# jgillick/genesis-forge

Hardware: AMD Instinct MI355X
Metric: env-steps/sec (higher is better)
Workload: dtype f32; 1 GPU; go2_12dof_full_manager_stack; num_envs_per_gpu=65536, global_num_envs=65536, dofs=12, reward_terms=6, termination_terms=2, command_managers=1, obs_width=48, scene=synthetic (gf_synth_scene_step), parallelism=env-shard x1, hsa_enable_ipc_mode_legacy=0, setup_steps_before_warmup=8, fused_post_physics=True, observation_output=fresh

## Files before the change

### genesis-forge_amd/csrc/gf_post.hip

```cpp
#include <dlfcn.h>

#include <atomic>
#include <cstdio>
#include <cstdlib>
#include <cstring>
#include <mutex>

#include "gf_post_args.h"
#include "gf_post_ws.h"
#include "gf_post_programs.h"

namespace gf {

static int cmd_slot_of_reward_op(int op) {
    switch (op) {
        case GF_R_CMD_TRACK_LIN_VEL:
        case GF_R_CMD_TRACK_ANG_VEL:
        case GF_R_STAND_STILL: return 0;
        case GF_R_FEET_AIR_TIME: return 1;
        default: return -1;
    }
}
static bool reward_op_has_contact(int op) { return op == GF_R_HAS_CONTACT || op == GF_R_CONTACT_FORCE || op == GF_R_FEET_AIR_TIME || op == GF_R_FEET_SLIDE; }
static bool term_op_has_contact(int op) { return op == GF_T_HAS_CONTACT || op == GF_T_CONTACT_FORCE || op == GF_T_CONTACT_FORCE_GRACE; }
// ... 506 lines not shown
    if (num_mgr > 0) {
        UNSUP(!post_program_folds(pk.a));
        rc = fold_contacts(pk, mgrs, num_mgr);
        if (rc) return rc;
    }
    return post_launch(pk.a, s);
}

}

extern "C" __attribute__((visibility("default"))) int gf_post_physics_check(const GfPostRefs* r) {
    gf::Packer pk;
    return gf::pack(r, pk);
}

using gf::lds_ws_floats;

namespace {
constexpr int kDynBase = 100, kDynMax = 256;
struct DynProgram {
    void* dl;
    char name[64];
    int (*matches)(const gf::GfPostArgs*);
    const void* kernel;
    size_t (*lds_bytes)(int, int);
    bool folds;
};
DynProgram g_dyn[kDynMax];
std::atomic<int> g_dyn_count{0};
std::mutex g_dyn_mutex;
// ... 93 lines not shown
#else
    const gf::GfPostArgs& a = packed;
#endif
    int omax = 0;
    for (int m = 0; m < a.n_obs; ++m) omax = a.obs[m].width > omax ? a.obs[m].width : omax;
    const size_t fold_lds = a.cfold.num_mgr > 0 ? gf::fold_lds_bytes(a.cfold.num_contacts) : 0;
    auto with_fold = [&](size_t bytes, bool interp) {
        const size_t need = fold_lds ? fold_lds + (interp ? sizeof(gf::GfPostArgs) : 0) : 0;
        return (bytes > need ? bytes : need) + (size_t)gf::kWsTilesLdsFloats * sizeof(float);
    };
    const unsigned grid = gf::env_grid(a.num_envs);
    if (prog < 0) prog = select_program(a);
    if (tick) {
        const dim3 tg(grid + (unsigned)tick->upkeep), tb(gf::kWsBlock);
#define GF_RUN_TICK(P, interp) \
        gf::klaunch(gf::post_ws_kernel_tick<P>, tg, tb, with_fold((interp ? sizeof(gf::GfPostArgs) : 0) + lds_ws_floats<P>(omax, a.n_gait) * sizeof(float), interp), s, a, *tick->act, *tick->scene, tick->upkeep)
        if (prog == 1) GF_RUN_TICK(gf::ProgGo2CommandDirection, false);
        else if (prog == 2) GF_RUN_TICK(gf::ProgGo2Simple, false);
        else if (a.num_dofs == 12) GF_RUN_TICK(GF_TICK_INTERP(3), true);
        else GF_RUN_TICK(GF_TICK_INTERP(7), true);
#undef GF_RUN_TICK
        return gf::launch_status();
    }
    gf::PhaseScope scope(GF_PHASE_POST, s);
    if (prog >= kDynBase) {
        const DynProgram& d = g_dyn[prog - kDynBase];
        const size_t lds_dyn = with_fold(d.lds_bytes(omax, a.n_gait), false);
        void* kargs[1] = {const_cast<gf::GfPostArgs*>(&a)};
        if (scope.active()) {
            scope.use_dispatch_events();
            (void)hipExtLaunchKernel(d.kernel, dim3(grid), dim3(gf::kWsBlock), kargs, lds_dyn, s, scope.start(), scope.stop(), 0);
// ... 80 lines not shown
```

### genesis-forge_amd/csrc/gf_post_programs.h

```cpp
#pragma once

#include "gf_post_ws.h"

namespace gf {

struct ProgGo2CommandDirection {
    static constexpr bool kStatic = true;
    static constexpr const char* name = "go2_command_direction";
    static constexpr int DV = 3;
    static constexpr int n_term = 2;
    static constexpr TermSig term[n_term] = {{GF_T_TIMEOUT, GF_TERM_FLAG_TIME_OUT}, {GF_T_BAD_ORIENTATION, 0}};
    static constexpr int n_rew = 6;
    static constexpr RewSig rew[n_rew] = {{GF_R_BASE_HEIGHT, 0, 0, 0},       {GF_R_CMD_TRACK_LIN_VEL, 0, 0, 0}, {GF_R_CMD_TRACK_ANG_VEL, 0, 0, 2},
                                          {GF_R_LIN_VEL_Z_L2, 0, 0, 0},      {GF_R_ACTION_RATE_L2, 0, 0, 0},    {GF_R_DOF_SIMILAR_TO_DEFAULT, 0, 0, 0}};
    static constexpr int n_cmd = 1;
    static constexpr int cmd_width[GF_POST_MAX_CMD] = {3, 0};
    static constexpr int n_obs = 1;
    static constexpr int obs_width[GF_POST_MAX_OBS] = {48, 0};
    static constexpr int obs_history[GF_POST_MAX_OBS] = {1, 0};
    static constexpr int obs_items[GF_POST_MAX_OBS] = {7, 0};
    static constexpr ItemSig item[GF_POST_MAX_OBS][kPostMaxItems] = {{{GF_O_COMMAND, 3, 0, false, false},
                                                                      {GF_O_ANG_VEL_BODY, 3, 0, false, false},
                                                                      {GF_O_LIN_VEL_BODY, 3, 0, false, false},
                                                                      {GF_O_PROJ_GRAVITY, 3, 0, false, false},
// ... 197 lines not shown
    static constexpr int n_cmd = 2;
    static constexpr int cmd_width[GF_POST_MAX_CMD] = {3, 1};
    static constexpr int n_obs = 2;
    static constexpr int obs_width[GF_POST_MAX_OBS] = {94, 61};
    static constexpr int obs_history[GF_POST_MAX_OBS] = {3, 1};
    static constexpr int obs_items[GF_POST_MAX_OBS] = {7, 4};
    static constexpr ItemSig item[GF_POST_MAX_OBS][kPostMaxItems] = {
        {{1, 1, 1, false, true}, {1, 3, 0, false, true}, {2, 3, 0, true, true}, {4, 3, 0, false, true}, {5, 28, 0, false, true}, {6, 28, 0, true, true}, {8, 28, 0, false, true}},
        {{10, 2, 1, true, false}, {3, 3, 0, false, false}, {7, 28, 0, false, false}, {9, 28, 0, false, false}}};
    static constexpr int n_air = 2;
    static constexpr int n_gait = 0;
};

template <class P>
inline size_t lds_ws_floats(int omax, int n_gait) {
    return (size_t)(x_fields(n_gait) + ws_sum_rows<P>() + ws_aux_rows<P>() + ws_pre_rows<P>() + ws_obs_norm_rows<P>()) * kEnvBlock + (size_t)(omax + 1) * kEnvBlock;
}

template <class P>
bool program_matches(const GfPostArgs& a) {
    if ((a.term_done != 0) != prog_term_done<P>::value || a.num_dofs != 4 * P::DV || a.num_term != P::n_term || (a.num_rew < 0 ? 0 : a.num_rew) != P::n_rew || a.n_cmd != P::n_cmd || a.n_obs != P::n_obs || a.n_air != P::n_air ||
        a.n_gait != P::n_gait)
        return false;
    for (int k = 0; k < P::n_term; ++k)
        if (a.tterms[k].op != P::term[k].op || a.tterms[k].flags != P::term[k].flags) return false;
    for (int k = 0; k < P::n_rew; ++k) {
        const GfTerm& t = a.rterms[k];
        if (t.op != P::rew[k].op || t.flags != P::rew[k].flags || t.i[0] != P::rew[k].i0 || t.i[1] != P::rew[k].i1) return false;
    }
    for (int c = 0; c < P::n_cmd; ++c)
        if (a.cmds[c].width != P::cmd_width[c]) return false;
// ... 42 lines not shown
```

### genesis-forge_amd/csrc/gf_post_ws.h

```cpp
#pragma once

#include <utility>

#include "gf_obs_hist.h"
#include "gf_post_args.h"
#include "gf_scene_tile.h"

namespace gf {

static_assert(kObsBlock == 4 * kEnvBlock, "the history helpers assume the 4-wave workgroup");
constexpr int kWsBlock = 4 * kEnvBlock;
enum : int { X_TERM = 0, X_TRUNC = 1, X_DONE = 2, X_BLIN = 3, X_BANG = 6, X_GRAV = 9, X_CMD = 12, X_DIRTY = 20, X_FIELDS = 21,
             X_GAIT = X_FIELDS  };
__host__ __device__ constexpr int x_fields(int n_gait) { return X_FIELDS + (n_gait > 0 ? GF_GAIT_ROW : 0); }

struct TermSig { int op, flags; };
struct RewSig { int op, flags, i0, i1; };
struct ItemSig { int op, width, i0; bool scaled, noisy; };

template <class P, class = void>
struct prog_term_done : std::false_type {};
template <class P>
struct prog_term_done<P, std::void_t<decltype(P::term_done)>> : std::bool_constant<P::term_done> {};

template <int DV_, bool TAIL_ = false>
struct Interp {
    static constexpr bool kStatic = false;
    static constexpr int DV = DV_;
    static constexpr bool kTail = TAIL_;
};

template <class P>
struct WithTick : P {
    static constexpr bool kTick = true;
};
template <class P, class = void>
struct prog_tick : std::false_type {};
template <class P>
struct prog_tick<P, std::void_t<decltype(P::kTick)>> : std::bool_constant<P::kTick> {};

template <class F, int... I>
__device__ __forceinline__ void static_for_impl(F&& f, std::integer_sequence<int, I...>) {
    (f(std::integral_constant<int, I>{}), ...);
}
template <int N, class F>
__device__ __forceinline__ void static_for(F&& f) {
    static_for_impl(f, std::make_integer_sequence<int, N>{});
}

template <class P>
__device__ __forceinline__ const GfPostArgs& pick_args(const GfPostArgs& k, const float* l) {
    if constexpr (P::kStatic) return k;
    else return *reinterpret_cast<const GfPostArgs*>(l);
}
// ... 73 lines not shown
}
template <class P>
__host__ __device__ constexpr bool ws_prog_folds() {
    if constexpr (P::kStatic) {
        if (P::n_term == 0 && P::n_rew == 0 && P::n_cmd == 0 && P::n_gait == 0) return false;
        if (P::n_air > 0) return true;
        for (int k = 0; k < P::n_term; ++k)
            if (term_op_counts_contacts(P::term[k].op)) return true;
        for (int k = 0; k < P::n_rew; ++k)
            if (reward_op_reads_contacts(P::rew[k].op)) return true;
        return ws_obs_has<P>(GF_O_CONTACT_FORCE_NORM);
    } else {
        return true;
    }
}

#ifndef GF_WS_AHEAD
#define GF_WS_AHEAD 0
#endif
constexpr int kWsTilesLdsFloats = GF_WS_AHEAD > 0 ? 4 * kEnvBlock : 0;

template <class P>
__device__ __forceinline__ void post_ws_body(const GfPostArgs& karg, const GfActionArgs* const tick_act, const GfSynthSceneArgs* const tick_scene,
                                             const int tick_upkeep) {
    constexpr int DV = P::DV;
    constexpr bool kTick = prog_tick<P>::value;
    unsigned ws_block = blockIdx.x;
    if constexpr (kTick) {
        if ((int)blockIdx.x < tick_upkeep) {
            action_upkeep(*tick_act, tick_upkeep, kWsBlock);
// ... 43 lines not shown
        n_term = P::n_term; n_rew = P::n_rew; n_cmd = P::n_cmd; n_obs = P::n_obs;
    } else {
        n_term = UNI(a.num_term); n_rew = UNI(a.num_rew); n_cmd = UNI(a.n_cmd); n_obs = UNI(a.n_obs);
    }
    const uint64_t seed = UNI(a.seed);
    const bool obs_only = UNI(a.obs_only) != 0;
    constexpr int R = DV;
    const uint32_t ro = e * (uint32_t)D;
    GfStepStats* const k_stats = UNI(a.stats);
    GfStepStats* shard = k_stats ? stats_shard(k_stats) : nullptr;
    const bool logging = UNI(a.logging) != 0;
    float* const k_sums = UNI(a.episode_sums);
    float* const k_reward = UNI(a.reward);
    const bool has_reward = n_rew >= 0 && k_reward != nullptr;
    const float4 z4 = make_float4(0.f, 0.f, 0.f, 0.f);
    if constexpr (kTick) {
        static_assert(GF_WS_AHEAD == 0, "the look-ahead experiment would pull rows of a tile whose tick has not run into this CU's L1");
        static_assert(kSynthTileBlock == kWsBlock && 3 * 3 * kEnvBlock <= X_FIELDS * kEnvBlock, "the tick's workgroup and LDS fit the kernel's");
        const GfSynthSceneArgs& sc = *tick_scene;
        const int rows = (int)((int64_t)sc.num_envs - n0 < kEnvBlock ? (int64_t)sc.num_envs - n0 : kEnvBlock);
        float (&s3)[3][kEnvBlock * 3] = *reinterpret_cast<float (*)[3][kEnvBlock * 3]>(xch);
        SynthBase ticked;
        synth_tick_tile<DV, kEnvBlock, true>(sc, *tick_act, n0, rows, s3, ticked);
        GF_WSTAMP(12);
        __syncthreads();
        GF_WSTAMP(13);
    }
#if GF_WS_AHEAD > 0
    {
        const int64_t next_id = tile_id + GF_WS_AHEAD;
        if (next_id < (N + kEnvBlock - 1) / kEnvBlock) {
            const int64_t n2 = next_id * kEnvBlock + lane;
            const uint32_t e2 = (uint32_t)(n2 < N ? n2 : N - 1), ro2 = e2 * (uint32_t)D;
            float* const pf = lds + kArgVec * 4 + wave * kEnvBlock;
            auto warm = [&](const bool on, const float* base, const uint32_t off) GF_INLINE_LAMBDA {
                __builtin_amdgcn_global_load_lds(gsel(on, base, off), pf, 4, 0, 0);
            };
            if (wave == 0) {
// ... 145 lines not shown
    int& gait_sel = ctl.gait_sel; int& gait_resampled = ctl.gait_resampled;
    if (wave == 0) {
        q = make_float4(1.f, 0.f, 0.f, 0.f);
        ep_len = 0; term = 0; trunc = 0;
#pragma unroll
        for (int j = 0; j < GF_GAIT_ROW; ++j) grow[j] = 0.f;
        gait_sel = 0; gait_resampled = 0;
        ctl.log_bits = 0u; ctl.gait_logged = 0;
    } else {
#pragma unroll
        for (int c = 0; c < DV; ++c) { r_a[c] = z4; r_b[c] = z4; r_c[c] = z4; }
    }

    float fold_w[kSumRows > 0 ? kSumRows : 1];
    int32_t fold_row[kSumRows > 0 ? kSumRows : 1];
    if (wave == 0) {
        q = ldg4(gsel((needs & PN_QUAT) != 0, UNI(a.quat), 4u * e));
        const GF_GLOBAL float* pp = gsel((needs & PN_POS) != 0, UNI(a.pos), 3u * e);
        const GF_GLOBAL float* lp = gsel((needs & PN_LIN) != 0, UNI(a.lin_vel), 3u * e);
        const GF_GLOBAL float* ap = gsel((needs & PN_ANG) != 0, UNI(a.ang_vel), 3u * e);
        const V3 pos{pp[0], pp[1], pp[2]};
        const V3 lin{lp[0], lp[1], lp[2]}, ang{ap[0], ap[1], ap[2]};
        ep_len = *gsel((needs & PN_EPLEN) != 0, UNI(a.episode_length), e);
        const int max_len = *gsel((needs & PN_MAXLEN) != 0, UNI(a.max_episode_length), e);
#pragma unroll
        for (int c = 0; c < GF_POST_MAX_CMD; ++c) {
            const bool on = c < n_cmd;
            const uint32_t w = on ? (uint32_t)UNI(cmd_row(c).width) : 0u;
            const GF_GLOBAL float* cp = gsel(on, on ? UNI(a.cmds[c].command) : nullptr, e * w);
#pragma unroll
            for (int j = 0; j < kPostMaxRanges; ++j) cmd[c][j] = cp[(uint32_t)j < w ? j : 0];
        }
        if (has_gait) {
            const GF_GLOBAL float* gp = G(UNI(a.gait.state)) + (int64_t)e * GF_GAIT_ROW;
            const float4 g0 = ldg4(gp), g1 = ldg4(gp + 4), g2 = ldg4(gp + 8), g3 = ldg4(gp + 12);
            grow[0] = g0.x; grow[1] = g0.y; grow[2] = g0.z; grow[3] = g0.w; grow[4] = g1.x; grow[5] = g1.y; grow[6] = g1.z; grow[7] = g1.w;
            grow[8] = g2.x; grow[9] = g2.y; grow[10] = g2.z; grow[11] = g2.w; grow[12] = g3.x; grow[13] = g3.y; grow[14] = g3.z; grow[15] = g3.w;
            gait_sel = (int)G(UNI(a.gait.selected))[e];
// ... 133 lines not shown
#pragma unroll
            for (int j = 0; j < kPostMaxRanges; ++j) xch[(X_CMD + c * kPostMaxRanges + j) * kEnvBlock + lane] = cmd[c][j];
        xch[X_DIRTY * kEnvBlock + lane] = (float)((cmd_dirty[0] ? 1 : 0) | (cmd_dirty[1] ? 2 : 0));
    } else if (wave == 1) {
        if (logging) {
            if constexpr (P::kStatic) {
                static_for<P::n_rew>([&](auto K) GF_INLINE_LAMBDA {
                    constexpr int k_ = decltype(K)::value;
                    __builtin_amdgcn_global_load_lds(k_sums + (int64_t)karg.rterms[k_].row * N + n, lds_sums + k_ * kEnvBlock, 4, 0, 0);
                });
            } else {
                for (int k = 0; k < n_rew; ++k)
                    __builtin_amdgcn_global_load_lds(k_sums + (int64_t)uni(a.rterms[k].row) * N + n, lds_sums + k * kEnvBlock, 4, 0, 0);
            }
        }
        const GF_GLOBAL float* p0 = gsel((needs & PN_DOFDEV) != 0, UNI(a.dof_pos), ro);
        const GF_GLOBAL float* p1 = gsel((needs & PN_ACTRATE) != 0, UNI(a.env_actions), ro);
        const GF_GLOBAL float* p2 = gsel((needs & PN_ACTRATE) != 0, UNI(a.env_last_actions), ro);
        const GF_GLOBAL float* p3 = gsel((needs & PN_DOFDEV) != 0, UNI(a.default_dof_pos), 0u);
        float4 r_def[R];
        row_load<DV>(r_a, p0, D); row_load<DV>(r_b, p1, D); row_load<DV>(r_c, p2, D); row_load<DV>(r_def, p3, D);
        const GF_GLOBAL float* pp = gsel((needs & PN_POS) != 0, UNI(a.pos), 3u * e);
        const V3 pos{pp[0], pp[1], pp[2]};
        float4 qb = make_float4(1.f, 0.f, 0.f, 0.f);
        V3 wlin{0.f, 0.f, 0.f}, wang{0.f, 0.f, 0.f};
        if constexpr (ws_rew_body_frame<P>()) {
            qb = ldg4(gsel((needs & PN_QUAT) != 0, UNI(a.quat), 4u * e));
            const GF_GLOBAL float* lp = gsel((needs & PN_LIN) != 0, UNI(a.lin_vel), 3u * e);
            const GF_GLOBAL float* ap = gsel((needs & PN_ANG) != 0, UNI(a.ang_vel), 3u * e);
            wlin = V3{lp[0], lp[1], lp[2]};
            wang = V3{ap[0], ap[1], ap[2]};
        }
        const float* k_secs = UNI(a.episode_seconds);
        const float secs_in = *gsel(has_reward && k_secs != nullptr, k_secs, e);
        float dof_dev = 0.f, act_rate = 0.f, cmd0[3];
        {
            const float* v0 = UNI(a.command[0].command);
            const bool nv = v0 != nullptr;
            const uint32_t w = nv ? (uint32_t)UNI(a.command[0].width) : 0u;
            const uint32_t st = nv ? (uint32_t)(UNI(a.command[0].stride) ? UNI(a.command[0].stride) : UNI(a.command[0].width)) : 0u;
            const GF_GLOBAL float* cp = gsel(nv, v0, e * st);
// ... 46 lines not shown
                });
            }
        }
        rew.pos = pos;
        rew.dof_dev = dof_dev; rew.act_rate = act_rate; rew.secs_in = secs_in;
        rew.cmd0[0] = cmd0[0]; rew.cmd0[1] = cmd0[1]; rew.cmd0[2] = cmd0[2];
        if constexpr (P::kStatic) {
            static_for<P::n_rew>([&](auto K) GF_INLINE_LAMBDA {
                constexpr int k_ = decltype(K)::value;
                rew.vals[k_] = vals[k_];
                fold_w[k_] = karg.rterms[k_].w; fold_row[k_] = karg.rterms[k_].row;
                asm volatile("" : "+s"(fold_w[k_]), "+s"(fold_row[k_]));
            });
        }
    } else if (wave == 2) {
        const GF_GLOBAL float* p0 = gsel((needs & PN_DOFPOS) != 0, UNI(a.dof_pos), ro);
        const GF_GLOBAL float* p1 = gsel((needs & PN_DOFVEL) != 0, UNI(a.dof_vel), ro);
        const float* k_def = UNI(a.default_dof_pos);
        const GF_GLOBAL float* p2 = gsel(k_def != nullptr, k_def, 0u);
        row_load<DV>(r_a, p0, D); row_load<DV>(r_b, p1, D); row_load<DV>(r_c, p2, D);
        GF_WSTAMP(9);
        if constexpr (kPreRows > 0) {
            RewardRegs rp;
            rp.pos = V3{0.f, 0.f, 0.f}; rp.blin = rp.pos; rp.bang = rp.pos; rp.grav = rp.pos;
            rp.dof_dev = 0.f; rp.act_rate = 0.f; rp.terminated = 0;
            rp.cmd0[0] = 0.f; rp.cmd0[1] = 0.f; rp.cmd0[2] = 0.f;
            rp.n = n; rp.live = live;
            static_for<P::n_rew>([&](auto K) GF_INLINE_LAMBDA {
                constexpr int k_ = decltype(K)::value;
                if constexpr (reward_op_memory_only(P::rew[k_].op)) {
                    GfTerm t = karg.rterms[k_];
                    t.op = P::rew[k_].op; t.flags = P::rew[k_].flags; t.i[0] = P::rew[k_].i0; t.i[1] = P::rew[k_].i1;
                    lds_pre[ws_pre_slot<P>(k_) * kEnvBlock + lane] = eval_reward_term(t, a, rp);
                }
            });
        }
    } else {
        const GF_GLOBAL float* p0 = gsel((needs & PN_TARGETS) != 0, UNI(a.targets), ro);
        const GF_GLOBAL float* p1 = gsel((needs & PN_ACTIONS) != 0, UNI(a.env_actions), ro);
        row_load<DV>(r_a, p0, D); row_load<DV>(r_b, p1, D);
        if constexpr (P::kStatic && ws_obs_has<P>(GF_O_DOF_FORCE)) {
            row_load<DV>(r_c, gsel(UNI(a.dof_force) != nullptr, UNI(a.dof_force), ro), D);
        }
        if constexpr (kNormRows > 0) {
            static_for<P::n_obs>([&](auto M) GF_INLINE_LAMBDA {
                constexpr int m_ = decltype(M)::value;
                static_for<P::obs_items[m_]>([&](auto I) GF_INLINE_LAMBDA {
                    constexpr int i_ = decltype(I)::value;
                    if constexpr (P::item[m_][i_].op == GF_O_CONTACT_FORCE_NORM) {
                        const GfContactView cv = a.contact[P::item[m_][i_].i0];
                        const GF_GLOBAL float* r = G(cv.contacts) + n * cv.num_links * 3;
#pragma unroll
                        for (int l = 0; l < P::item[m_][i_].width; ++l)
                            lds_norm[(ws_obs_norm_slot<P>(m_, i_) + l) * kEnvBlock + lane] = norm3(r[3 * l], r[3 * l + 1], r[3 * l + 2]);
                    }
// ... 473 lines not shown
```

### genesis-forge_amd/csrc/gf_scene_tile.h

```cpp
#pragma once

#include "gf_action_row.h"

namespace gf {

struct SynthBase {
    float p[3], q[4], v[3], w[3];
};

struct SynthDraws {
    U4 b0, b1;
};
__device__ __forceinline__ SynthDraws synth_draws(const GfSynthSceneArgs& a, const uint32_t genv) {
    return SynthDraws{philox4x32_10(genv, 0u, (uint32_t)a.tick, (uint32_t)(a.tick >> 32), (uint32_t)a.seed, (uint32_t)(a.seed >> 32)),
                      philox4x32_10(genv, 1u, (uint32_t)a.tick, (uint32_t)(a.tick >> 32), (uint32_t)a.seed, (uint32_t)(a.seed >> 32))};
}

__device__ __forceinline__ void synth_base_math(const GfSynthSceneArgs& a, const float4 q4, const V3 w0, const V3 v0, const V3 p0,
                                                const SynthDraws& r, SynthBase& out) {
    const float dt = a.dt;
    const U4 b0 = r.b0, b1 = r.b1;
    const float s[6] = {u24_to_unit(b0.x) * 2.0f - 1.0f, u24_to_unit(b0.y) * 2.0f - 1.0f, u24_to_unit(b0.z) * 2.0f - 1.0f,
                        u24_to_unit(b0.w) * 2.0f - 1.0f, u24_to_unit(b1.x) * 2.0f - 1.0f, u24_to_unit(b1.y) * 2.0f - 1.0f};
    float w[3] = {w0.x, w0.y, w0.z}, v[3] = {v0.x, v0.y, v0.z}, p[3] = {p0.x, p0.y, p0.z};
// ... 18 lines not shown
    for (int j = 0; j < 3; ++j) { out.w[j] = w[j]; out.v[j] = v[j]; out.p[j] = p[j]; }
#pragma unroll
    for (int j = 0; j < 4; ++j) out.q[j] = nq[j];
}

__device__ __forceinline__ void synth_joint(float t, float& p, float& v, float rate, float dt) {
    v = (t - p) * rate;
    p = p + v * dt;
}

constexpr int kSynthTileBlock = 256;
constexpr int kSynthDofLanes = kSynthTileBlock - GF_WAVE;

__device__ __forceinline__ void wave_lds_sync() { __builtin_amdgcn_wave_barrier(); }

template <int DV, int TE, bool FOLD = false>
__device__ __forceinline__ void synth_dof_tile(const GfSynthSceneArgs& a, const GfActionArgs& act, const int64_t n0, const int rows, const int t) {
    const float dt = a.dt, rate = a.joint_rate;
    if constexpr (FOLD) {
        static_assert(DV > 0, "the fold moves float4s");
        constexpr int kIt = (TE * (DV > 0 ? DV : 1) + kSynthDofLanes - 1) / kSynthDofLanes;
        const int cnt = rows * DV;
        const int64_t f0 = n0 * DV;
        const float4* x4 = reinterpret_cast<const float4*>(act.actions_in) + f0;
        const bool keep = act.env_actions != nullptr;
        float4* e4 = reinterpret_cast<float4*>(keep ? act.env_actions : act.targets) + f0;
        float4* l4 = reinterpret_cast<float4*>(keep ? act.env_last_actions : act.targets) + f0;
        float4* t4 = reinterpret_cast<float4*>(act.targets) + f0;
        float4* p4 = reinterpret_cast<float4*>(a.dof_pos) + f0;
        float4* v4 = reinterpret_cast<float4*>(a.dof_vel) + f0;
        const int mode = act.mode;
        int flags = 0;
// ... 15 lines not shown
            if constexpr (!kConstsFirst) c0 = action_consts4(act, 4 * ((i < cnt ? i : cnt - 1) % DV), mode);
            float4 last, actions, tg;
            int fl = 0;
            action_row4(act, c0, mode, x[k], pv[k], last, actions, tg, fl);
            float4 v, p = dp[k];
            synth_joint(tg.x, p.x, v.x, rate, dt);
            synth_joint(tg.y, p.y, v.y, rate, dt);
            synth_joint(tg.z, p.z, v.z, rate, dt);
            synth_joint(tg.w, p.w, v.w, rate, dt);
            if (i < cnt) {
                flags |= fl;
                if (keep) { l4[i] = last; e4[i] = actions; }
                t4[i] = tg;
                v4[i] = v;
                p4[i] = p;
            }
        }
        action_flags_commit(act, flags);
    } else if (DV > 0) {
        constexpr int kIt = DV > 0 ? (TE * DV + kSynthDofLanes - 1) / kSynthDofLanes : 1;
        const int cnt = rows * DV;
        const float4* t4 = reinterpret_cast<const float4*>(a.targets) + n0 * DV;
        float4* p4 = reinterpret_cast<float4*>(a.dof_pos) + n0 * DV;
        float4* v4 = reinterpret_cast<float4*>(a.dof_vel) + n0 * DV;
        float4 tg[kIt], dp[kIt];
#pragma unroll
        for (int k = 0; k < kIt; ++k) {
            const int i = t + k * kSynthDofLanes;
            if (i < cnt) { tg[k] = t4[i]; dp[k] = p4[i]; }
        }
// ... 10 lines not shown
                p4[i] = p;
            }
        }
    } else {
        const int64_t base = n0 * a.num_dofs;
        const int cnt = rows * a.num_dofs;
        for (int i = t; i < cnt; i += kSynthDofLanes) {
            float p = a.dof_pos[base + i], v;
            synth_joint(a.targets[base + i], p, v, rate, dt);
            a.dof_vel[base + i] = v;
            a.dof_pos[base + i] = p;
        }
    }
}

template <int TE, bool FOLD = false>
__device__ __forceinline__ void synth_base_tile(const GfSynthSceneArgs& a, const GfActionArgs& act, const int64_t n0, const int rows, const int lane,
                                                float (&s3)[3][TE * 3], SynthBase& out) {
    constexpr int kJ = (TE * 3 + GF_WAVE - 1) / GF_WAVE;
    const int cnt = rows * 3;
    float* const pos = a.pos + n0 * 3;
    float* const lin = a.lin_vel + n0 * 3;
    float* const ang = a.ang_vel + n0 * 3;
    float xp[kJ], xv[kJ], xw[kJ];
#pragma unroll
    for (int j = 0; j < kJ; ++j) {
        const int i = lane + j * GF_WAVE < cnt ? lane + j * GF_WAVE : cnt - 1;
        xp[j] = pos[i]; xv[j] = lin[i]; xw[j] = ang[i];
    }
    const bool mine = lane < rows;
    const float4 q4 = load_quat(a.quat, n0 + (mine ? lane : rows - 1));
    int32_t ep = 0;
    if constexpr (FOLD) {
// ... 14 lines not shown
    const V3 v0{s3[1][3 * e], s3[1][3 * e + 1], s3[1][3 * e + 2]};
    const V3 w0{s3[2][3 * e], s3[2][3 * e + 1], s3[2][3 * e + 2]};
    synth_base_math(a, q4, w0, v0, p0, r, out);
    wave_lds_sync();
    if (mine) {
#pragma unroll
        for (int j = 0; j < 3; ++j) { s3[0][3 * lane + j] = out.p[j]; s3[1][3 * lane + j] = out.v[j]; s3[2][3 * lane + j] = out.w[j]; }
    }
    wave_lds_sync();
#pragma unroll
    for (int j = 0; j < kJ; ++j) {
        const int i = lane + j * GF_WAVE;
        const float yp = s3[0][i < TE * 3 ? i : 0], yv = s3[1][i < TE * 3 ? i : 0], yw = s3[2][i < TE * 3 ? i : 0];
        if (i < cnt) { pos[i] = yp; lin[i] = yv; ang[i] = yw; }
    }
    if (mine) reinterpret_cast<float4*>(a.quat)[n0 + lane] = make_float4(out.q[0], out.q[1], out.q[2], out.q[3]);
    if constexpr (FOLD) {
        if (mine && act.episode_length) act.episode_length[n0 + lane] = ep + 1;
    }
}

template <int DV, int TE, bool FOLD = false>
__device__ __forceinline__ void synth_tick_tile(const GfSynthSceneArgs& a, const GfActionArgs& act, const int64_t n0, const int rows,
                                                float (&s3)[3][TE * 3], SynthBase& b) {
    const int tid = threadIdx.x;
    if (tid >= GF_WAVE) synth_dof_tile<DV, TE, FOLD>(a, act, n0, rows, tid - GF_WAVE);
    else synth_base_tile<TE, FOLD>(a, act, n0, rows, tid, s3, b);
}

}
```

### genesis-forge_amd/genesis_forge_amd/_native.py

```python
from __future__ import annotations

import ctypes as C
import os
from typing import Optional

GF_ABI_VERSION = 8
GF_MAX_TERMS = 24
GF_MAX_TERM_TERMS = 16
GF_MAX_OBS_ITEMS = 24
GF_MAX_CONTACT_VIEWS = 4
GF_MAX_COMMAND_VIEWS = 4
GF_MAX_EXT = 16
GF_MAX_LINK_IDS = 32
GF_MAX_RANGES = 8
GF_MAX_OBS_WIDTH = 256
GF_MAX_GAITS = 4
GF_STATS_SHARDS = 64

GF_ACTION_POSITION, GF_ACTION_WITHIN_LIMITS = 0, 1

GF_T_TIMEOUT = 1
GF_T_BAD_ORIENTATION = 2
GF_T_BASE_HEIGHT_BELOW = 3
GF_T_OUT_OF_BOUNDS = 4
# ... 557 lines not shown
        if os.environ.get("GF_NO_CHAIN", "0") == "1":
            self.lib.gf_set_option(GF_OPT_CHAIN, 0)
        if os.environ.get("GF_GRAPH", "0") == "1":
            self.lib.gf_set_option(GF_OPT_GRAPH, 1)
            self.graph_enabled = True
        self.lib.gf_stats_pack.restype = C.c_int
        self.lib.gf_stats_pack.argtypes = [C.POINTER(GfStatsPackArgs), C.c_void_p]
        self.lib.gf_stats_last_reset.restype = C.c_int
        self.lib.gf_stats_last_reset.argtypes = [C.c_void_p, C.c_int, C.c_void_p, C.c_void_p]
        self.lib.gf_post_physics_check.restype = C.c_int
        self.lib.gf_post_physics_check.argtypes = [C.POINTER(GfPostRefs)]
        self.lib.gf_post_physics_step_contacts.restype = C.c_int
        self.lib.gf_post_physics_step_contacts.argtypes = [C.POINTER(GfPostRefs), C.POINTER(C.c_void_p), C.c_int, C.c_void_p]
        self.lib.gf_post_physics_describe.restype = C.c_int
        self.lib.gf_post_physics_describe.argtypes = [C.POINTER(GfPostRefs), C.c_char_p, C.c_int]
        self.lib.gf_post_program_register.restype = C.c_int
        self.lib.gf_post_program_register.argtypes = [C.c_char_p, C.POINTER(C.c_int)]
        self.lib.gf_event_create.restype = C.c_void_p
        self.lib.gf_event_synchronize.restype = C.c_int
        self.lib.gf_event_synchronize.argtypes = [C.c_void_p]
        self.lib.gf_set_option.restype = C.c_int
        self.lib.gf_set_option.argtypes = [C.c_int, C.c_int]
        self.lib.gf_profile_begin.restype = C.c_int
        self.lib.gf_profile_begin.argtypes = [C.c_int, C.c_int]
        variant = os.environ.get("GF_POST_VARIANT")
        if variant is not None:
            self.set_option(GF_OPT_POST_VARIANT, int(variant))
        self.lib.gf_profile_end.restype = C.c_int
        self.lib.gf_profile_end.argtypes = [C.POINTER(C.c_double), C.POINTER(C.c_int)]
        n = self.lib.gf_sizeof(GF_SIZEOF_MINIBATCH)
# ... 86 lines not shown

    def post_check(self, refs) -> bool:
        return self.lib.gf_post_physics_check(C.byref(refs)) == 0

    def post_step_contacts(self, refs, contact_args: list) -> int:
        arr = (C.c_void_p * max(1, len(contact_args)))(*[C.addressof(a) for a in contact_args])
        return self.lib.gf_post_physics_step_contacts(C.byref(refs), arr, len(contact_args), self._stream())

    def post_describe(self, refs) -> str:
        buf = C.create_string_buffer(4096)
        rc = self.lib.gf_post_physics_describe(C.byref(refs), buf, len(buf))
        if rc != 0:
            self._raise("post_physics_describe", rc)
        return buf.value.decode()

    def register_program(self, plugin_path: str) -> int:
        pid = C.c_int(-1)
        rc = self.lib.gf_post_program_register(plugin_path.encode(), C.byref(pid))
        if rc != 0:
            self._raise(f"post_program_register({plugin_path})", rc)
        return pid.value

    def stats_pack(self, src_ptr: int, dst_ptr: int) -> None:
        a = GfStatsPackArgs()
        a.src, a.dst = src_ptr, dst_ptr
        rc = self.lib.gf_stats_pack(C.byref(a), self._stream())
        if rc != 0:
            self._raise("stats_pack", rc)

    def stats_last_reset(self, rows_ptr: int, num_rows: int, dst_ptr: int) -> None:
# ... 57 lines not shown
```

### include/gf_step.h

```cpp
#ifndef GF_STEP_H
#define GF_STEP_H

#include <stdint.h>

#ifdef __cplusplus
extern "C" {
#endif

#define GF_ABI_VERSION 8

#define GF_MAX_TERMS 24
#define GF_MAX_TERM_TERMS 16
#define GF_MAX_OBS_ITEMS 24
#define GF_MAX_CONTACT_VIEWS 4
#define GF_MAX_COMMAND_VIEWS 4
#define GF_MAX_EXT 16
#define GF_MAX_LINK_IDS 32
#define GF_MAX_RANGES 8
#define GF_MAX_OBS_WIDTH 256
#define GF_MAX_GAITS 4

#define GF_OK 0
#define GF_E_NULL (-1)
#define GF_E_RANGE (-2)
// ... 719 lines not shown
    const GfCommandArgs* command_step[GF_POST_MAX_CMD];
    const GfCommandArgs* command_reset[GF_POST_MAX_CMD];
    const GfObservationArgs* observe[GF_POST_MAX_OBS];
    int32_t num_gait;
    int32_t flags;
    const GfGaitArgs* gait_step[GF_POST_MAX_GAIT];
    const GfGaitArgs* gait_reset[GF_POST_MAX_GAIT];
    uint8_t* gait_flags_next[GF_POST_MAX_GAIT];
    const GfRolloutArgs* rollout;
} GfPostRefs;

int gf_post_physics_check(const GfPostRefs* r);
int gf_post_physics_step(const GfPostRefs* r, void* stream);
int gf_post_physics_step_contacts(const GfPostRefs* r, const GfContactArgs* const* contacts, int num_contacts, void* stream);
int gf_post_physics_describe(const GfPostRefs* r, char* buf, int cap);
int gf_post_program_register(const char* plugin_path, int* program_id_out);
int gf_post_program_count(void);

typedef struct GfOp {
    int32_t phase;
    int32_t _pad;
    const void* args;
} GfOp;

enum { GF_OP_STATS_CLEAR = 100, GF_OP_STATS_COPY = 101, GF_OP_POST_PHYSICS = 102 ,
       GF_OP_STATS_PACK = 103  };

#define GF_STATS_VECTOR_LEN (GF_MAX_TERM_TERMS + 5 + GF_MAX_TERMS + GF_MAX_GAITS)
typedef struct GfStatsPackArgs {
    const GfStepStats* src;
// ... 66 lines not shown
```

Measured before the change: 5.368 billion env-steps/s.

## Hand ticked scene state to post-physics waves through LDS instead of global reloads

In the fused tick+post kernel, the synthetic scene tick now writes the freshly computed dof rows (pos, vel, targets, actions, last actions), base pose/velocities and episode length into LDS through a sink. The post-physics waves then read them from LDS instead of reloading from global memory. This removes a round trip through L2/HBM for data the same workgroup just produced, at the cost of more LDS per workgroup, which may reduce occupancy. It also adds a host API that exposes the needs bitmask.

New measurement: 5.760 billion env-steps/s (median of 6 runs). +7.3%, better.

```diff
diff --git a/genesis-forge_amd/csrc/gf_post.hip b/genesis-forge_amd/csrc/gf_post.hip
--- a/genesis-forge_amd/csrc/gf_post.hip
+++ b/genesis-forge_amd/csrc/gf_post.hip
@@ -544,6 +544,20 @@
     return gf::pack(r, pk);
 }
 
+static_assert(gf::PN_POS == GF_POST_NEEDS_POS && gf::PN_QUAT == GF_POST_NEEDS_QUAT && gf::PN_LIN == GF_POST_NEEDS_LIN && gf::PN_ANG == GF_POST_NEEDS_ANG &&
+              gf::PN_DOFPOS == GF_POST_NEEDS_DOFPOS && gf::PN_DOFVEL == GF_POST_NEEDS_DOFVEL && gf::PN_TARGETS == GF_POST_NEEDS_TARGETS &&
+              gf::PN_ACTIONS == GF_POST_NEEDS_ACTIONS && gf::PN_LAST == GF_POST_NEEDS_LAST && gf::PN_EPLEN == GF_POST_NEEDS_EPLEN &&
+              gf::PN_MAXLEN == GF_POST_NEEDS_MAXLEN && gf::PN_DOFDEV == GF_POST_NEEDS_DOFDEV && gf::PN_ACTRATE == GF_POST_NEEDS_ACTRATE &&
+              gf::PN_DOFFORCE == GF_POST_NEEDS_DOFFORCE, "gf_step.h names the kernel's bits");
+extern "C" __attribute__((visibility("default"))) int gf_post_physics_needs(const GfPostRefs* r, uint32_t* needs_out) {
+    if (!needs_out) return GF_E_NULL;
+    gf::Packer pk;
+    const int rc = gf::pack(r, pk);
+    if (rc) return rc;
+    *needs_out = pk.a.needs;
+    return GF_OK;
+}
+
 using gf::lds_ws_floats;
 
 namespace {
@@ -667,7 +681,7 @@
     if (tick) {
         const dim3 tg(grid + (unsigned)tick->upkeep), tb(gf::kWsBlock);
 #define GF_RUN_TICK(P, interp) \
-        gf::klaunch(gf::post_ws_kernel_tick<P>, tg, tb, with_fold((interp ? sizeof(gf::GfPostArgs) : 0) + lds_ws_floats<P>(omax, a.n_gait) * sizeof(float), interp), s, a, *tick->act, *tick->scene, tick->upkeep)
+        gf::klaunch(gf::post_ws_kernel_tick<P>, tg, tb, with_fold((interp ? sizeof(gf::GfPostArgs) : 0) + lds_ws_floats<gf::WithTick<P>>(omax, a.n_gait) * sizeof(float), interp), s, a, *tick->act, *tick->scene, tick->upkeep)
         if (prog == 1) GF_RUN_TICK(gf::ProgGo2CommandDirection, false);
         else if (prog == 2) GF_RUN_TICK(gf::ProgGo2Simple, false);
         else if (a.num_dofs == 12) GF_RUN_TICK(GF_TICK_INTERP(3), true);
diff --git a/genesis-forge_amd/csrc/gf_post_programs.h b/genesis-forge_amd/csrc/gf_post_programs.h
--- a/genesis-forge_amd/csrc/gf_post_programs.h
+++ b/genesis-forge_amd/csrc/gf_post_programs.h
@@ -235,7 +235,10 @@
 
 template <class P>
 inline size_t lds_ws_floats(int omax, int n_gait) {
-    return (size_t)(x_fields(n_gait) + ws_sum_rows<P>() + ws_aux_rows<P>() + ws_pre_rows<P>() + ws_obs_norm_rows<P>()) * kEnvBlock + (size_t)(omax + 1) * kEnvBlock;
+    const size_t front = (size_t)(x_fields(n_gait) + ws_sum_rows<P>()) * kEnvBlock;
+    const size_t back = (size_t)(ws_aux_rows<P>() + ws_pre_rows<P>() + ws_obs_norm_rows<P>()) * kEnvBlock + (size_t)(omax + 1) * kEnvBlock;
+    if constexpr (ws_hands_over<P>()) return front + (back > (size_t)ws_hand_floats<P>() ? back : (size_t)ws_hand_floats<P>());
+    else return front + back;
 }
 
 template <class P>
diff --git a/genesis-forge_amd/csrc/gf_post_ws.h b/genesis-forge_amd/csrc/gf_post_ws.h
--- a/genesis-forge_amd/csrc/gf_post_ws.h
+++ b/genesis-forge_amd/csrc/gf_post_ws.h
@@ -38,6 +38,25 @@
 struct prog_tick : std::false_type {};
 template <class P>
 struct prog_tick<P, std::void_t<decltype(P::kTick)>> : std::bool_constant<P::kTick> {};
+
+enum : int { H_DOFPOS = 0, H_DOFVEL = 1, H_TARGETS = 2, H_ACTIONS = 3, H_LAST = 4, H_STREAMS = 5 };
+enum : int { HB_POS = 0, HB_QUAT = 3, HB_LIN = 7, HB_ANG = 10, HB_EPLEN = 13, HB_FIELDS = 14 };
+template <int DV, int TE>
+struct TickHand {
+    float4* rows;
+    float* base_rows;
+    __device__ __forceinline__ void dof(const int i, const float4& last, const float4& actions, const float4& tg, const float4& v, const float4& p) const {
+        rows[H_DOFPOS * TE * DV + i] = p; rows[H_DOFVEL * TE * DV + i] = v; rows[H_TARGETS * TE * DV + i] = tg;
+        rows[H_ACTIONS * TE * DV + i] = actions; rows[H_LAST * TE * DV + i] = last;
+    }
+    __device__ __forceinline__ void base(const int e, const SynthBase& b) const {
+#pragma unroll
+        for (int j = 0; j < 3; ++j) { base_rows[(HB_POS + j) * TE + e] = b.p[j]; base_rows[(HB_LIN + j) * TE + e] = b.v[j]; base_rows[(HB_ANG + j) * TE + e] = b.w[j]; }
+#pragma unroll
+        for (int j = 0; j < 4; ++j) base_rows[(HB_QUAT + j) * TE + e] = b.q[j];
+    }
+    __device__ __forceinline__ void episode(const int e, const int32_t len) const { base_rows[HB_EPLEN * TE + e] = __builtin_bit_cast(float, len); }
+};
 
 template <class F, int... I>
 __device__ __forceinline__ void static_for_impl(F&& f, std::integer_sequence<int, I...>) {
@@ -141,6 +160,15 @@
         return true;
     }
 }
+
+template <class P>
+__host__ __device__ constexpr bool ws_hands_over() {
+    if constexpr (!prog_tick<P>::value) return false;
+    else if constexpr (P::kStatic) return ws_pre_rows<P>() == 0 && ws_obs_norm_rows<P>() == 0;
+    else return P::DV == 3 && !P::kTail;
+}
+template <class P>
+__host__ __device__ constexpr int ws_hand_floats() { return H_STREAMS * kEnvBlock * 4 * P::DV + HB_FIELDS * kEnvBlock + 4 * P::DV; }
 
 #ifndef GF_WS_AHEAD
 #define GF_WS_AHEAD 0
@@ -214,6 +242,11 @@
     float* const k_reward = UNI(a.reward);
     const bool has_reward = n_rew >= 0 && k_reward != nullptr;
     const float4 z4 = make_float4(0.f, 0.f, 0.f, 0.f);
+    constexpr bool kHand = ws_hands_over<P>();
+    float4* const hand_rows = reinterpret_cast<float4*>(lds_aux);
+    float* const hand_base = lds_aux + H_STREAMS * kEnvBlock * 4 * DV;
+    float4* const hand_zero = reinterpret_cast<float4*>(hand_base + HB_FIELDS * kEnvBlock);
+    int hand_env = lane;
     if constexpr (kTick) {
         static_assert(GF_WS_AHEAD == 0, "the look-ahead experiment would pull rows of a tile whose tick has not run into this CU's L1");
         static_assert(kSynthTileBlock == kWsBlock && 3 * 3 * kEnvBlock <= X_FIELDS * kEnvBlock, "the tick's workgroup and LDS fit the kernel's");
@@ -221,7 +254,14 @@
         const int rows = (int)((int64_t)sc.num_envs - n0 < kEnvBlock ? (int64_t)sc.num_envs - n0 : kEnvBlock);
         float (&s3)[3][kEnvBlock * 3] = *reinterpret_cast<float (*)[3][kEnvBlock * 3]>(xch);
         SynthBase ticked;
-        synth_tick_tile<DV, kEnvBlock, true>(sc, *tick_act, n0, rows, s3, ticked);
+        if constexpr (kHand) {
+            static_assert(kPreRows == 0 && kNormRows == 0, "the handed rows run from the scratch rows into the observation tile");
+            synth_tick_tile<DV, kEnvBlock, true>(sc, *tick_act, n0, rows, s3, ticked, TickHand<DV, kEnvBlock>{hand_rows, hand_base});
+            hand_env = lane < rows ? lane : rows - 1;
+            if (threadIdx.x < DV) hand_zero[threadIdx.x] = z4;
+        } else {
+            synth_tick_tile<DV, kEnvBlock, true>(sc, *tick_act, n0, rows, s3, ticked);
+        }
         GF_WSTAMP(12);
         __syncthreads();
         GF_WSTAMP(13);
@@ -397,14 +437,36 @@
 
     float fold_w[kSumRows > 0 ? kSumRows : 1];
     int32_t fold_row[kSumRows > 0 ? kSumRows : 1];
+    auto hand_row = [&](float4 (&r)[R], const bool on, const int stream) GF_INLINE_LAMBDA {
+        const float4* const src = on ? hand_rows + stream * kEnvBlock * DV + hand_env * DV : hand_zero;
+#pragma unroll
+        for (int c = 0; c < DV; ++c) r[c] = src[c];
+    };
+    auto hand_v3 = [&](const bool on, const int field) GF_INLINE_LAMBDA {
+        const float* const h = hand_base + field * kEnvBlock + hand_env;
+        return on ? V3{h[0], h[kEnvBlock], h[2 * kEnvBlock]} : V3{0.f, 0.f, 0.f};
+    };
+    auto hand_quat = [&](const bool on) GF_INLINE_LAMBDA {
+        const float* const h = hand_base + HB_QUAT * kEnvBlock + hand_env;
+        return on ? make_float4(h[0], h[kEnvBlock], h[2 * kEnvBlock], h[3 * kEnvBlock]) : z4;
+    };
     if (wave == 0) {
-        q = ldg4(gsel((needs & PN_QUAT) != 0, UNI(a.quat), 4u * e));
-        const GF_GLOBAL float* pp = gsel((needs & PN_POS) != 0, UNI(a.pos), 3u * e);
-        const GF_GLOBAL float* lp = gsel((needs & PN_LIN) != 0, UNI(a.lin_vel), 3u * e);
-        const GF_GLOBAL float* ap = gsel((needs & PN_ANG) != 0, UNI(a.ang_vel), 3u * e);
-        const V3 pos{pp[0], pp[1], pp[2]};
-        const V3 lin{lp[0], lp[1], lp[2]}, ang{ap[0], ap[1], ap[2]};
-        ep_len = *gsel((needs & PN_EPLEN) != 0, UNI(a.episode_length), e);
+        V3 pos, lin, ang;
+        if constexpr (kHand) {
+            q = hand_quat((needs & PN_QUAT) != 0);
+            pos = hand_v3((needs & PN_POS) != 0, HB_POS);
+            lin = hand_v3((needs & PN_LIN) != 0, HB_LIN);
+            ang = hand_v3((needs & PN_ANG) != 0, HB_ANG);
+            ep_len = (needs & PN_EPLEN) != 0 ? __builtin_bit_cast(int, hand_base[HB_EPLEN * kEnvBlock + hand_env]) : 0;
+        } else {
+            q = ldg4(gsel((needs & PN_QUAT) != 0, UNI(a.quat), 4u * e));
+            const GF_GLOBAL float* pp = gsel((needs & PN_POS) != 0, UNI(a.pos), 3u * e);
+            const GF_GLOBAL float* lp = gsel((needs & PN_LIN) != 0, UNI(a.lin_vel), 3u * e);
+            const GF_GLOBAL float* ap = gsel((needs & PN_ANG) != 0, UNI(a.ang_vel), 3u * e);
+            pos = V3{pp[0], pp[1], pp[2]};
+            lin = V3{lp[0], lp[1], lp[2]}; ang = V3{ap[0], ap[1], ap[2]};
+            ep_len = *gsel((needs & PN_EPLEN) != 0, UNI(a.episode_length), e);
+        }
         const int max_len = *gsel((needs & PN_MAXLEN) != 0, UNI(a.max_episode_length), e);
 #pragma unroll
         for (int c = 0; c < GF_POST_MAX_CMD; ++c) {
@@ -568,17 +630,28 @@
                     __builtin_amdgcn_global_load_lds(k_sums + (int64_t)uni(a.rterms[k].row) * N + n, lds_sums + k * kEnvBlock, 4, 0, 0);
             }
         }
-        const GF_GLOBAL float* p0 = gsel((needs & PN_DOFDEV) != 0, UNI(a.dof_pos), ro);
-        const GF_GLOBAL float* p1 = gsel((needs & PN_ACTRATE) != 0, UNI(a.env_actions), ro);
-        const GF_GLOBAL float* p2 = gsel((needs & PN_ACTRATE) != 0, UNI(a.env_last_actions), ro);
         const GF_GLOBAL float* p3 = gsel((needs & PN_DOFDEV) != 0, UNI(a.default_dof_pos), 0u);
         float4 r_def[R];
-        row_load<DV>(r_a, p0, D); row_load<DV>(r_b, p1, D); row_load<DV>(r_c, p2, D); row_load<DV>(r_def, p3, D);
-        const GF_GLOBAL float* pp = gsel((needs & PN_POS) != 0, UNI(a.pos), 3u * e);
-        const V3 pos{pp[0], pp[1], pp[2]};
+        V3 pos;
+        if constexpr (kHand) {
+            row_load<DV>(r_def, p3, D);
+            hand_row(r_a, (needs & PN_DOFDEV) != 0, H_DOFPOS); hand_row(r_b, (needs & PN_ACTRATE) != 0, H_ACTIONS); hand_row(r_c, (needs & PN_ACTRATE) != 0, H_LAST);
+            pos = hand_v3((needs & PN_POS) != 0, HB_POS);
+        } else {
+            const GF_GLOBAL float* p0 = gsel((needs & PN_DOFDEV) != 0, UNI(a.dof_pos), ro);
+            const GF_GLOBAL float* p1 = gsel((needs & PN_ACTRATE) != 0, UNI(a.env_actions), ro);
+            const GF_GLOBAL float* p2 = gsel((needs & PN_ACTRATE) != 0, UNI(a.env_last_actions), ro);
+            row_load<DV>(r_a, p0, D); row_load<DV>(r_b, p1, D); row_load<DV>(r_c, p2, D); row_load<DV>(r_def, p3, D);
+            const GF_GLOBAL float* pp = gsel((needs & PN_POS) != 0, UNI(a.pos), 3u * e);
+            pos = V3{pp[0], pp[1], pp[2]};
+        }
         float4 qb = make_float4(1.f, 0.f, 0.f, 0.f);
         V3 wlin{0.f, 0.f, 0.f}, wang{0.f, 0.f, 0.f};
-        if constexpr (ws_rew_body_frame<P>()) {
+        if constexpr (ws_rew_body_frame<P>() && kHand) {
+            qb = hand_quat((needs & PN_QUAT) != 0);
+            wlin = hand_v3((needs & PN_LIN) != 0, HB_LIN);
+            wang = hand_v3((needs & PN_ANG) != 0, HB_ANG);
+        } else if constexpr (ws_rew_body_frame<P>()) {
             qb = ldg4(gsel((needs & PN_QUAT) != 0, UNI(a.quat), 4u * e));
             const GF_GLOBAL float* lp = gsel((needs & PN_LIN) != 0, UNI(a.lin_vel), 3u * e);
             const GF_GLOBAL float* ap = gsel((needs & PN_ANG) != 0, UNI(a.ang_vel), 3u * e);
@@ -655,11 +728,16 @@
             });
         }
     } else if (wave == 2) {
-        const GF_GLOBAL float* p0 = gsel((needs & PN_DOFPOS) != 0, UNI(a.dof_pos), ro);
-        const GF_GLOBAL float* p1 = gsel((needs & PN_DOFVEL) != 0, UNI(a.dof_vel), ro);
         const float* k_def = UNI(a.default_dof_pos);
         const GF_GLOBAL float* p2 = gsel(k_def != nullptr, k_def, 0u);
-        row_load<DV>(r_a, p0, D); row_load<DV>(r_b, p1, D); row_load<DV>(r_c, p2, D);
+        if constexpr (kHand) {
+            hand_row(r_a, (needs & PN_DOFPOS) != 0, H_DOFPOS); hand_row(r_b, (needs & PN_DOFVEL) != 0, H_DOFVEL);
+        } else {
+            const GF_GLOBAL float* p0 = gsel((needs & PN_DOFPOS) != 0, UNI(a.dof_pos), ro);
+            const GF_GLOBAL float* p1 = gsel((needs & PN_DOFVEL) != 0, UNI(a.dof_vel), ro);
+            row_load<DV>(r_a, p0, D); row_load<DV>(r_b, p1, D);
+        }
+        row_load<DV>(r_c, p2, D);
         GF_WSTAMP(9);
         if constexpr (kPreRows > 0) {
             RewardRegs rp;
@@ -677,9 +755,13 @@
             });
         }
     } else {
-        const GF_GLOBAL float* p0 = gsel((needs & PN_TARGETS) != 0, UNI(a.targets), ro);
-        const GF_GLOBAL float* p1 = gsel((needs & PN_ACTIONS) != 0, UNI(a.env_actions), ro);
-        row_load<DV>(r_a, p0, D); row_load<DV>(r_b, p1, D);
+        if constexpr (kHand) {
+            hand_row(r_a, (needs & PN_TARGETS) != 0, H_TARGETS); hand_row(r_b, (needs & PN_ACTIONS) != 0, H_ACTIONS);
+        } else {
+            const GF_GLOBAL float* p0 = gsel((needs & PN_TARGETS) != 0, UNI(a.targets), ro);
+            const GF_GLOBAL float* p1 = gsel((needs & PN_ACTIONS) != 0, UNI(a.env_actions), ro);
+            row_load<DV>(r_a, p0, D); row_load<DV>(r_b, p1, D);
+        }
         if constexpr (P::kStatic && ws_obs_has<P>(GF_O_DOF_FORCE)) {
             row_load<DV>(r_c, gsel(UNI(a.dof_force) != nullptr, UNI(a.dof_force), ro), D);
         }
diff --git a/genesis-forge_amd/csrc/gf_scene_tile.h b/genesis-forge_amd/csrc/gf_scene_tile.h
--- a/genesis-forge_amd/csrc/gf_scene_tile.h
+++ b/genesis-forge_amd/csrc/gf_scene_tile.h
@@ -56,8 +56,15 @@
 
 __device__ __forceinline__ void wave_lds_sync() { __builtin_amdgcn_wave_barrier(); }
 
-template <int DV, int TE, bool FOLD = false>
-__device__ __forceinline__ void synth_dof_tile(const GfSynthSceneArgs& a, const GfActionArgs& act, const int64_t n0, const int rows, const int t) {
+struct SynthNoSink {
+    __device__ __forceinline__ void dof(int, const float4&, const float4&, const float4&, const float4&, const float4&) const {}
+    __device__ __forceinline__ void base(int, const SynthBase&) const {}
+    __device__ __forceinline__ void episode(int, int32_t) const {}
+};
+
+template <int DV, int TE, bool FOLD = false, class Sink = SynthNoSink>
+__device__ __forceinline__ void synth_dof_tile(const GfSynthSceneArgs& a, const GfActionArgs& act, const int64_t n0, const int rows, const int t,
+                                               const Sink& sink = Sink{}) {
     const float dt = a.dt, rate = a.joint_rate;
     if constexpr (FOLD) {
         static_assert(DV > 0, "the fold moves float4s");
@@ -103,6 +110,7 @@
                 t4[i] = tg;
                 v4[i] = v;
                 p4[i] = p;
+                sink.dof(i, last, actions, tg, v, p);
             }
         }
         action_flags_commit(act, flags);
@@ -143,9 +151,9 @@
     }
 }
 
-template <int TE, bool FOLD = false>
+template <int TE, bool FOLD = false, class Sink = SynthNoSink>
 __device__ __forceinline__ void synth_base_tile(const GfSynthSceneArgs& a, const GfActionArgs& act, const int64_t n0, const int rows, const int lane,
-                                                float (&s3)[3][TE * 3], SynthBase& out) {
+                                                float (&s3)[3][TE * 3], SynthBase& out, const Sink& sink = Sink{}) {
     constexpr int kJ = (TE * 3 + GF_WAVE - 1) / GF_WAVE;
     const int cnt = rows * 3;
     float* const pos = a.pos + n0 * 3;
@@ -190,18 +198,22 @@
         const float yp = s3[0][i < TE * 3 ? i : 0], yv = s3[1][i < TE * 3 ? i : 0], yw = s3[2][i < TE * 3 ? i : 0];
         if (i < cnt) { pos[i] = yp; lin[i] = yv; ang[i] = yw; }
     }
-    if (mine) reinterpret_cast<float4*>(a.quat)[n0 + lane] = make_float4(out.q[0], out.q[1], out.q[2], out.q[3]);
+    if (mine) {
+        reinterpret_cast<float4*>(a.quat)[n0 + lane] = make_float4(out.q[0], out.q[1], out.q[2], out.q[3]);
+        sink.base(lane, out);
+    }
     if constexpr (FOLD) {
         if (mine && act.episode_length) act.episode_length[n0 + lane] = ep + 1;
-    }
-}
-
-template <int DV, int TE, bool FOLD = false>
+        if (mine) sink.episode(lane, ep + 1);
+    }
+}
+
+template <int DV, int TE, bool FOLD = false, class Sink = SynthNoSink>
 __device__ __forceinline__ void synth_tick_tile(const GfSynthSceneArgs& a, const GfActionArgs& act, const int64_t n0, const int rows,
-                                                float (&s3)[3][TE * 3], SynthBase& b) {
+                                                float (&s3)[3][TE * 3], SynthBase& b, const Sink& sink = Sink{}) {
     const int tid = threadIdx.x;
-    if (tid >= GF_WAVE) synth_dof_tile<DV, TE, FOLD>(a, act, n0, rows, tid - GF_WAVE);
-    else synth_base_tile<TE, FOLD>(a, act, n0, rows, tid, s3, b);
-}
-
-}
+    if (tid >= GF_WAVE) synth_dof_tile<DV, TE, FOLD>(a, act, n0, rows, tid - GF_WAVE, sink);
+    else synth_base_tile<TE, FOLD>(a, act, n0, rows, tid, s3, b, sink);
+}
+
+}
diff --git a/genesis-forge_amd/genesis_forge_amd/_native.py b/genesis-forge_amd/genesis_forge_amd/_native.py
--- a/genesis-forge_amd/genesis_forge_amd/_native.py
+++ b/genesis-forge_amd/genesis_forge_amd/_native.py
@@ -595,6 +595,8 @@
         self.lib.gf_post_physics_step_contacts.argtypes = [C.POINTER(GfPostRefs), C.POINTER(C.c_void_p), C.c_int, C.c_void_p]
         self.lib.gf_post_physics_describe.restype = C.c_int
         self.lib.gf_post_physics_describe.argtypes = [C.POINTER(GfPostRefs), C.c_char_p, C.c_int]
+        self.lib.gf_post_physics_needs.restype = C.c_int
+        self.lib.gf_post_physics_needs.argtypes = [C.POINTER(GfPostRefs), C.POINTER(C.c_uint32)]
         self.lib.gf_post_program_register.restype = C.c_int
         self.lib.gf_post_program_register.argtypes = [C.c_char_p, C.POINTER(C.c_int)]
         self.lib.gf_event_create.restype = C.c_void_p
@@ -711,6 +713,13 @@
             self._raise("post_physics_describe", rc)
         return buf.value.decode()
 
+    def post_needs(self, refs) -> int:
+        word = C.c_uint32(0)
+        rc = self.lib.gf_post_physics_needs(C.byref(refs), C.byref(word))
+        if rc != 0:
+            self._raise("post_physics_needs", rc)
+        return int(word.value)
+
     def register_program(self, plugin_path: str) -> int:
         pid = C.c_int(-1)
         rc = self.lib.gf_post_program_register(plugin_path.encode(), C.byref(pid))
diff --git a/include/gf_step.h b/include/gf_step.h
--- a/include/gf_step.h
+++ b/include/gf_step.h
@@ -757,6 +757,11 @@
 int gf_post_physics_step(const GfPostRefs* r, void* stream);
 int gf_post_physics_step_contacts(const GfPostRefs* r, const GfContactArgs* const* contacts, int num_contacts, void* stream);
 int gf_post_physics_describe(const GfPostRefs* r, char* buf, int cap);
+enum { GF_POST_NEEDS_POS = 1, GF_POST_NEEDS_QUAT = 2, GF_POST_NEEDS_LIN = 4, GF_POST_NEEDS_ANG = 8, GF_POST_NEEDS_DOFPOS = 16,
+       GF_POST_NEEDS_DOFVEL = 32, GF_POST_NEEDS_TARGETS = 64, GF_POST_NEEDS_ACTIONS = 128, GF_POST_NEEDS_LAST = 256,
+       GF_POST_NEEDS_EPLEN = 512, GF_POST_NEEDS_MAXLEN = 1024, GF_POST_NEEDS_DOFDEV = 2048 ,
+       GF_POST_NEEDS_ACTRATE = 4096 , GF_POST_NEEDS_DOFFORCE = 8192 };
+int gf_post_physics_needs(const GfPostRefs* r, uint32_t* needs_out);
 int gf_post_program_register(const char* plugin_path, int* program_id_out);
 int gf_post_program_count(void);
 
```
